# CycloneBoy/pdf_table

Measured on AMD Instinct MI355X. Metric: pages/s, higher is better.
Workload: dtype bf16

## Files before the change

include/pdftable_hip.h:

```cpp
#ifndef PDFTABLE_HIP_H
#define PDFTABLE_HIP_H

#include <stddef.h>
#include <stdint.h>

#ifdef __cplusplus
extern "C" {
#endif

#define PT_OK 0
#define PT_ERR_INVALID 1
#define PT_ERR_HIP 2
#define PT_ERR_STATE 3
#define PT_ERR_FORMAT 4

typedef struct pt_engine pt_engine;
typedef void* pt_stream;

int pt_engine_create(int device_id, pt_engine** out);
void pt_engine_destroy(pt_engine* e);
const char* pt_last_error(void);
int pt_abi_version(void);
int pt_engine_check(pt_engine* e);
int pt_engine_set_lstm_cluster(pt_engine* e, int on);
// ... 151 lines not shown
                  const float* d_cr, const float* d_reg, int n, int h, int w, int wiz_rev, float vis_thresh,
                  int32_t* d_counts, float* d_dets, float* d_logi, pt_stream stream);

int pt_tsr_forward_decode(pt_engine* e, const uint16_t* d_input_bf16, int n, int in_h, int in_w, int wiz_rev,
                          float vis_thresh, int32_t* d_counts, float* d_dets, float* d_logi, pt_stream stream);

int pt_centernet_forward_net(pt_engine* e, const uint16_t* d_input_bf16, int n, int H, int W, float* d_hm, float* d_v2c, float* d_c2v,
                             float* d_reg, pt_stream stream);

#define PT_CENTERNET_MAX_CELLS 1000
int pt_centernet_decode(pt_engine* e, const float* d_hm, const float* d_v2c, const float* d_c2v, const float* d_reg, int n, int h, int w,
                        const double* d_affine, int32_t* d_counts, float* d_cells, pt_stream stream);

int pt_tsr_process(pt_engine* e, const float* d_logi, const float* d_dets, const int32_t* h_counts, int n_tables,
                   int use_2dpe, float* d_logic, float* d_stacked, pt_stream stream);

int pt_op_conv2d(pt_engine* e, const uint16_t* d_in, int B, int H, int W, int Cin, const uint16_t* d_w_tiled,
                 const float* d_bias, int N, int ks, int stride, uint16_t* d_out, int out_cstride, int out_coff,
                 int rep, int shuffle_cout, const uint16_t* d_res, int res_mode, int relu, int split, int out_lo_off,
                 pt_stream stream);
int pt_op_conv1x1_ex(pt_engine* e, const uint16_t* d_in, int B, int H, int W, int Cin, const uint16_t* d_w_tiled, const float* d_bias,
                     int N, uint16_t* d_out, float* d_out_f32, int out_cstride, int n_valid, const float* d_res_f32, int relu,
                     const int32_t* d_ylimit, pt_stream stream);

int pt_op_dcn(pt_engine* e, const uint16_t* d_in, const float* d_om, int B, int H, int W, int C, const uint16_t* d_w_tiled,
              const float* d_bias, int N, uint16_t* d_out, int relu, int split, pt_stream stream);

int pt_op_stem7x7(pt_engine* e, const uint16_t* d_in, int B, int H, int W, const uint16_t* d_w, const float* d_bias,
                  uint16_t* d_out, int split, pt_stream stream);
int pt_op_maxpool3x3s2(pt_engine* e, const uint16_t* d_in, int B, int H, int W, int C, uint16_t* d_out, int split,
                       pt_stream stream);
int pt_op_db_head_final(pt_engine* e, const uint16_t* d_in, int B, int H, int W, const void* d_w, const float* d_bias,
                        float* d_prob, float* d_logits, int split, pt_stream stream);

int pt_op_dwconv(pt_engine* e, const uint16_t* d_in, int B, int H, int W, int C, const float* d_w_taps, const float* d_bias, int k,
                 int stride, int act, uint16_t* d_out, int split, pt_stream stream);
int pt_op_add(pt_engine* e, const uint16_t* d_a, const uint16_t* d_b, uint16_t* d_out, long long npix, int C, int split, pt_stream stream);
int pt_op_maxpool(pt_engine* e, const uint16_t* d_in, int B, int H, int W, int C, int k, int stride, int pad, uint16_t* d_out,
                  int split, pt_stream stream);
int pt_op_avgpool(pt_engine* e, const uint16_t* d_in, int B, int H, int W, int C, int k, uint16_t* d_out, int split, pt_stream stream);
int pt_op_chan_mean(pt_engine* e, const uint16_t* d_in, int B, int HW, int C, float* d_scratch, uint16_t* d_mean, int split, pt_stream stream);
int pt_op_chan_mean_scratch_floats(int B, int C);
int pt_op_scale_channels(pt_engine* e, const uint16_t* d_in, const uint16_t* d_gate, int B, int HW, int C, uint16_t* d_out,
                         int split, pt_stream stream);
int pt_op_act(pt_engine* e, const uint16_t* d_in, long long n_elems, int kind, float alpha, float beta, uint16_t* d_out, int C, int split,
              pt_stream stream);
// ... 73 lines not shown
```

pdf_table_amd/csrc/api_common.cpp:

```cpp
#include <stdarg.h>
#include <stdio.h>

#include "../../include/pdftable_hip.h"

static thread_local char g_err[1024] = "";

void pt_set_error(const char* fmt, ...) {
  va_list ap;
  va_start(ap, fmt);
  vsnprintf(g_err, sizeof(g_err), fmt, ap);
  va_end(ap);
}

extern "C" {

const char* pt_last_error(void) { return g_err; }

int pt_abi_version(void) { return 17; }

}
```

pdf_table_amd/csrc/c_api.hip:

```cpp
#include <stdarg.h>
#include <stdio.h>
#include <stdlib.h>

#include <cmath>

#include "common.h"

namespace PT_FMT_NS {
namespace api {

static int ensure(void** buf, size_t* cap, size_t need);

int pt_engine_check(pt_engine* e) {
  PT_REQUIRE(e, "pt_engine_check: null engine");
  if (e->lstm_err && *e->lstm_err) {
    *e->lstm_err = 0;
    e->lstm_cluster = 0;
    pt_set_error("lstm_cluster_kernel: a workgroup waited > 2^22 polls for its peers -- the launch was not co-resident "
                 "(GPU shared with another process or stream?).  The recognition results since the last check are invalid; "
                 "this engine now uses the streaming LSTM kernel (pt_engine_set_lstm_cluster(e, 0)): run the batch again");
    return PT_ERR_HIP;
  }
  return PT_OK;
}
// ... 910 lines not shown
                 const float* d_bias, int N, int ks, int stride, uint16_t* d_out, int out_cstride, int out_coff,
                 int rep, int shuffle_cout, const uint16_t* d_res, int res_mode, int relu, int split, int out_lo_off,
                 pt_stream stream) {
  PT_REQUIRE(e != nullptr, "pt_op_conv2d: null engine");
  ConvDesc d;
  d.in = d_in; d.B = B; d.H = H; d.W = W; d.Cin = Cin; d.w = d_w_tiled; d.bias = d_bias; d.N = N; d.ks = ks;
  d.stride = stride; d.out = d_out; d.out_cstride = out_cstride; d.out_coff = out_coff; d.rep = rep;
  d.shuffle_cout = shuffle_cout; d.res = d_res; d.res_mode = res_mode; d.relu = relu;
  d.split = split; d.out_lo_off = out_lo_off;
  return pt_launch_conv(e, d, reinterpret_cast<hipStream_t>(stream));
}

int pt_op_conv1x1_ex(pt_engine* e, const uint16_t* d_in, int B, int H, int W, int Cin, const uint16_t* d_w_tiled, const float* d_bias,
                     int N, uint16_t* d_out, float* d_out_f32, int out_cstride, int n_valid, const float* d_res_f32, int relu,
                     const int32_t* d_ylimit, pt_stream stream) {
  PT_REQUIRE(e != nullptr, "pt_op_conv1x1_ex: null engine");
  ConvDesc d;
  d.in = d_in; d.B = B; d.H = H; d.W = W; d.Cin = Cin; d.w = d_w_tiled; d.bias = d_bias; d.N = N; d.ks = 1; d.stride = 1;
  d.out = d_out_f32 ? nullptr : d_out; d.out_f32 = d_out_f32; d.out_cstride = out_cstride; d.n_valid = n_valid; d.res_f32 = d_res_f32;
  d.relu = relu; d.ylimit = d_ylimit;
  return pt_launch_conv(e, d, reinterpret_cast<hipStream_t>(stream));
}

int pt_op_stem7x7(pt_engine* e, const uint16_t* d_in, int B, int H, int W, const uint16_t* d_w, const float* d_bias,
                  uint16_t* d_out, int split, pt_stream stream) {
  PT_REQUIRE(e != nullptr, "pt_op_stem7x7: null engine");
  return pt_launch_stem7x7(e, d_in, B, H, W, d_w, d_bias, d_out, split, reinterpret_cast<hipStream_t>(stream));
}

int pt_op_maxpool3x3s2(pt_engine* e, const uint16_t* d_in, int B, int H, int W, int C, uint16_t* d_out, int split,
                       pt_stream stream) {
  PT_REQUIRE(e && d_in && d_out, "pt_op_maxpool3x3s2: bad arguments");
  return pt_launch_maxpool3x3s2(d_in, B, H, W, C, d_out, split, reinterpret_cast<hipStream_t>(stream));
}

int pt_op_db_head_final(pt_engine* e, const uint16_t* d_in, int B, int H, int W, const void* d_w, const float* d_bias,
                        float* d_prob, float* d_logits, int split, pt_stream stream) {
  PT_REQUIRE(e && d_in && d_w && d_bias && (d_prob || d_logits), "pt_op_db_head_final: bad arguments");
  return pt_launch_db_head_final(d_in, B, H, W, d_w, d_bias, d_prob, d_logits, split, reinterpret_cast<hipStream_t>(stream));
}

int pt_op_dcn(pt_engine* e, const uint16_t* d_in, const float* d_om, int B, int H, int W, int C, const uint16_t* d_w_tiled,
              const float* d_bias, int N, uint16_t* d_out, int relu, int split, pt_stream stream) {
  PT_REQUIRE(e && d_in && d_om && d_w_tiled && d_bias && d_out, "pt_op_dcn: null argument");
  PT_REQUIRE(B > 0 && H > 0 && W > 0, "pt_op_dcn: empty map (B=%d H=%d W=%d)", B, H, W);
  return pt_launch_dcn_fused(e, d_in, d_om, d_w_tiled, d_bias, d_out, B, H, W, C, N, split, relu, reinterpret_cast<hipStream_t>(stream));
// ... 86 lines not shown
```

pdf_table_amd/csrc/common.h:

```cpp
#pragma once
#include <hip/hip_runtime.h>
#include <stdint.h>
#include <string.h>

#include <map>
#include <string>
#include <vector>

#include "../../include/pdftable_hip.h"
#include "act16.h"

typedef uint16_t bf16_t;

void pt_set_error(const char* fmt, ...);

#define PT_HIP_CHECK(expr)                                                                  \
  do {                                                                                      \
    hipError_t _e = (expr);                                                                 \
    if (_e != hipSuccess) {                                                                 \
      pt_set_error("%s failed: %s (%s:%d)", #expr, hipGetErrorString(_e), __FILE__, __LINE__); \
      return PT_ERR_HIP;                                                                    \
    }                                                                                       \
  } while (0)

// ... 200 lines not shown
  const float* slope = nullptr;
  int pool = 0;
  const int* ylimit = nullptr;
  const int* xlimit = nullptr;
  const int* xlimit_cols = nullptr;
  const int* xlimit_rows = nullptr;
  const int* block_list = nullptr;
  int split = 0;
  int out_lo_off = 0;
  const void* head_w = nullptr;
  const float* head_b = nullptr;
  float* head_prob = nullptr;
  float* head_logits = nullptr;
  float* argmax_part = nullptr;
  int n_valid = 0;
  float* out_f32 = nullptr;
  const float* res_f32 = nullptr;
  unsigned tap_mask[8] = {0, 0, 0, 0, 0, 0, 0, 0};
  int xp_store = 0;
  int alg_n = 0;
  double alg_scale = 1.0;
};
int pt_launch_conv(pt_engine* e, const ConvDesc& d, hipStream_t s);
int pt_launch_crnn_conv01(pt_engine* e, const bf16_t* gray, int n, const float* w64x9, const float* b0, const bf16_t* w1, const float* b1, bf16_t* p1,
                          const int* xlimit, const int* xlimit_cols, hipStream_t s);
int pt_launch_dwpw(pt_engine* e, const bf16_t* in, int B, int H, int W, int C, const float* dw_w, const float* dw_b, int k, int stride, int dw_act,
                   const ConvDesc& pw, hipStream_t s);

int pt_launch_stem7x7(pt_engine* e, const bf16_t* in, int B, int H, int W, const bf16_t* w, const float* bias,
                      bf16_t* out, int split, hipStream_t s, int stride = 2, int n_valid = 0);

int pt_launch_det_preprocess(const uint8_t* pages, int n, int h, int w, int nh, int nw, int flavour, int split,
                             bf16_t* out, hipStream_t s);
int pt_launch_dcn_fused(pt_engine* e, const bf16_t* x, const float* om, const bf16_t* w, const float* bias, bf16_t* out,
                        int B, int H, int W, int C, int N, int split, int relu, hipStream_t s, const bf16_t* omw = nullptr, const float* omb = nullptr);
bool pt_dcn_fuses_om(const pt_engine* e, int C, int split);
int pt_launch_maxpool3x3s2(const bf16_t* in, int B, int H, int W, int C, bf16_t* out, int split, hipStream_t s);
int pt_launch_stem7x7_pool(pt_engine* e, const bf16_t* in, int B, int H, int W, const bf16_t* w, const float* bias, bf16_t* out,
                           hipStream_t s);
int pt_launch_db_head_final(const bf16_t* in, int B, int H, int W, const void* w4x64, const float* bias, float* prob,
                            float* logits, int split, hipStream_t s);
int pt_launch_db_head_mfma(const bf16_t* in, int B, int H, int W, const bf16_t* w3, const float* b3, const bf16_t* w6,
                           const float* b6, float* prob, float* logits, hipStream_t s, uint32_t* bitmap = nullptr, float thresh = 0.f);
int pt_launch_bitmap(const float* prob, int n, int H, int W, float thresh, int dilate, uint32_t* bitmap,
                     hipStream_t s);
int pt_launch_box_scores(const float* prob, int n, int H, int W, const float* boxes, int nb, float* scores,
// ... 149 lines not shown
```

pdf_table_amd/csrc/conv_igemm.hip:

```cpp
#include <stdio.h>
#include <stdlib.h>

#include <type_traits>

#include "common.h"

namespace PT_FMT_NS {

typedef __attribute__((ext_vector_type(8))) __bf16 bf16x8;
typedef __attribute__((ext_vector_type(8))) _Float16 f16x8;
typedef __attribute__((ext_vector_type(16))) float f32x16;
typedef __attribute__((ext_vector_type(4))) float f32x4;
typedef __attribute__((ext_vector_type(4))) uint32_t u32x4;
typedef __attribute__((ext_vector_type(2))) uint32_t u32x2;

struct ConvK {
  const bf16_t* in;
  const bf16_t* w;
  const float* bias;
  bf16_t* out;
  const bf16_t* res;
  int B, H, W, Cin, Ho, Wo, N;
  int out_cstride, out_coff, rep, shuffle_cout, res_mode, relu;
  int tiles_x, tiles_y, n_tiles;
// ... 1289 lines not shown
            stage[((rbase + m) * 32 + tx) * 64 + n * 32 + lx] = acc[m][n][r];
          }
    }
    __syncthreads();
    if constexpr (C::NBLK > 1) {
      static_assert(NT == 2 || C::NBLK == 1, "blocked tiles: one pass = all rows of one 64-channel half");
#pragma unroll 1
      for (int j = 0; j < C::NBLK; ++j) {
        int bj = blk_b[0], xj = blk_x[0];
#pragma unroll
        for (int t = 1; t < C::NBLK; ++t)
          if (j == t) { bj = blk_b[t]; xj = blk_x[t]; }
        if (xj < p.Wo) epilogue_store<C::BR, 32, C::NTHR, 2>(p, stage + j * C::BR * 32 * 64, tid, bj, 0, xj, (nb * 2 + pass) * 64);
      }
    } else if (NT == 1) {
      epilogue_store<C::PASS_ROWS, 32, C::NTHR, 0>(p, stage, tid, b, oy0 + C::PASS_ROWS * pass, ox0, nb * 64);
    } else {
      epilogue_store<C::PASS_ROWS, 32, C::NTHR, 0>(p, stage, tid, b, oy0, ox0, (nb * 2 + pass) * 64);
    }
  }
#endif
}

template <int NT, int NWV, int S>
__global__ __launch_bounds__(64 * NWV, 2) void conv3x3_pipe_persist_kernel(ConvK p) {
#if defined(__HIP_DEVICE_COMPILE__)
  a16_kernel_enter();
  using C = PipeCfg<NT, NWV, 0, S>;
  static_assert(C::NBLK == 1, "ordinary tiles");
  extern __shared__ __attribute__((aligned(16))) char smem[];
  const int tid = threadIdx.x;
  const int lane = tid & 63;
  const int wave = __builtin_amdgcn_readfirstlane(tid >> 6);
  const int lx = lane & 31, qh = lane >> 5;
  const int wm = NT == 1 ? wave : (wave >> 1);
  const int wn = NT == 1 ? 0 : (wave & 1);
  const int G = gridDim.x;
  const int Lw = xcd_remap(blockIdx.x, G);
  const int t0 = (int)((long long)Lw * p.total_tiles / G), t1 = (int)((long long)(Lw + 1) * p.total_tiles / G);
  if (t0 >= t1) return;
  const int in_cs = p.Cin;
  const int nch32 = p.Cin >> 5, nslices = nch32 * 2;

  constexpr int OOB = 0x7FFFF000;
  int meta[C::SLOTS];
  bool is_in[C::SLOTS];
  int dst[C::SLOTS];
#pragma unroll
  for (int j = 0; j < C::SLOTS; ++j) {
    int k = wave + NWV * j;
    if (k >= C::T_INSTR) k = C::T_INSTR - 1;
    is_in[j] = k < C::IN_INSTR;
    dst[j] = k * 1024;
    if (is_in[j]) {
      const int U = k * 64 + lane;
      const int pix = U >> 1;
      const int pr = pix / C::TWIN, sx = pix - pr * C::TWIN;
      const int q = (U & 1) ^ ((sx >> 3) & 1);
      const int ix = S == 1 ? sx : (sx < C::XEVEN ? 2 * sx : 2 * (sx - C::XEVEN) + 1);
      meta[j] = U < C::IN_UNITS ? (pr | (ix << 8) | (q << 16)) : -1;
    } else {
      const int U = (k - C::IN_INSTR) * 64 + lane;
// ... 102 lines not shown
      __syncthreads();
      if constexpr (!LAST) load_frags(smem + (P ^ 1) * C::BUF_BYTES, 0, ((P + 1) * NTAP) & 1);
      mma_tap((P * NTAP + NTAP - 1) & 1);
      tap_groups<LAST ? 0 : 2 + C::MT, 2 * C::MT, 0>();
    };
    for (int c = 0; c + 2 < nslices; c += 2) {
      skew_slice(c, std::integral_constant<int, 0>{}, std::false_type{}, in_off(c + 1), w_off(c + 1));
      skew_slice(c + 1, std::integral_constant<int, 1>{}, std::false_type{}, in_off(c + 2), w_off(c + 2));
    }
    skew_slice(nslices - 2, std::integral_constant<int, 0>{}, std::false_type{}, in_off(nslices - 1), w_off(nslices - 1));
    const Tile done = cur;
    {
      const bool has_next = ti + 1 < t1;
      cur = decode(has_next ? ti + 1 : ti);
      offsets(cur, vo);
      if (!has_next) {
#pragma unroll
        for (int j = 0; j < C::SLOTS; ++j) vo[j] = OOB;
      }
      r_in = rsrc_in(cur);
      r_w = rsrc_w(cur);
    }
    skew_slice(nslices - 1, std::integral_constant<int, 1>{}, std::true_type{}, 0, 0);
    {
      const int n0 = (NT == 1 ? done.nb : done.nb * 2 + wn) * 64;
      const DirectBias bs = direct_bias<2>(p, n0, qh);
#pragma unroll
      for (int m = 0; m < C::MT; ++m) {
        epilogue_direct_row<2>(p, acc[m], bs, done.b, done.oy0 + C::MT * wm + m, done.ox0, lx, n0, qh, nullptr);
#pragma unroll
        for (int n = 0; n < 2; ++n)
#pragma unroll
          for (int r = 0; r < 16; ++r) acc[m][n][r] = 0.f;
      }
    }
    load_frags(smem, 0, 0);
  }
#endif
}

struct GemmPipeCfg {
  static constexpr int NWV = 8, NTHR = 512, MT = 4, NG = 16;
  static constexpr int KS = 64, NW = 128;
  static constexpr int A_BYTES = NG * 32 * KS * 2, W_BYTES = NW * KS * 2, BUF_BYTES = A_BYTES + W_BYTES;
  static constexpr int A_INSTR = A_BYTES / 1024, W_INSTR = W_BYTES / 1024, SLOTS = (A_INSTR + W_INSTR) / NWV;
  static constexpr int SMEM = 2 * BUF_BYTES;
  static_assert(A_INSTR % NWV == 0 && W_INSTR % NWV == 0, "a slot is an A or a W request for every wave alike");
};

template <bool LIST>
__global__ __launch_bounds__(512, 2) void gemm_pipe_kernel(ConvK p) {
#if defined(__HIP_DEVICE_COMPILE__)
  a16_kernel_enter();
  using C = GemmPipeCfg;
  extern __shared__ __attribute__((aligned(16))) char smem[];
  const int tid = threadIdx.x;
  const int lane = tid & 63;
  const int wave = __builtin_amdgcn_readfirstlane(tid >> 6);
  const int lx = lane & 31, qh = lane >> 5;
  const int wm = wave >> 1, wn = wave & 1;

// ... 1435 lines not shown
  k.n_tiles = k.N / C::NW;
  k.tiles_x = (k.Wo + C::TW - 1) / C::TW;
  k.tiles_y = (k.Ho + C::TH - 1) / C::TH;
  const long long total = (long long)k.B * k.tiles_x * k.tiles_y * k.n_tiles;
  PT_REQUIRE(total > 0 && total < (1ll << 31), "conv grid out of range (%lld tiles)", total);
  k.total_tiles = (int)total;
  const int per_cu = 2 * C::BUF_BYTES <= 80 * 1024 ? 2 : 1;
  long long grid = (long long)e->num_cu * per_cu;
  if (const char* gv = getenv("PT_CONV_PERSIST_GRID")) {
    const int gg = atoi(gv);
    if (gg > 0) grid = gg;
  }
  if (grid > total) grid = total;
  char label[48];
  snprintf(label, sizeof(label), "conv3x3 %sv5%s %d->%d @%dx%d", S == 2 ? "s2 " : "", NWV == 4 ? "h" : "", k.Cin, k.N, k.Ho, k.Wo);
  {
    PtProfScope prof(e, s, PT_PROF_CONV3X3, flop, label);
    hipLaunchKernelGGL((conv3x3_pipe_persist_kernel<NT, NWV, S>), dim3((unsigned)grid), dim3(C::NTHR), 2 * C::BUF_BYTES, s, k);
  }
  PT_HIP_CHECK(hipGetLastError());
  return PT_OK;
}

static int launch_gemm_pipe(pt_engine* e, ConvK& k, hipStream_t s, double flop) {
  using C = GemmPipeCfg;
  static bool attr_done = false;
  if (!attr_done) {
    PT_HIP_CHECK(hipFuncSetAttribute(reinterpret_cast<const void*>(&gemm_pipe_kernel<false>), hipFuncAttributeMaxDynamicSharedMemorySize, C::SMEM));
    PT_HIP_CHECK(hipFuncSetAttribute(reinterpret_cast<const void*>(&gemm_pipe_kernel<true>), hipFuncAttributeMaxDynamicSharedMemorySize, C::SMEM));
    attr_done = true;
  }
  const long long M = (long long)k.B * k.H * k.W, groups = M / 32;
  {
    const char* xv = getenv("PT_GEMM_XP");
    k.xp_store = !(xv && xv[0] == '0') && !k.out_f32;
  }
  k.n_tiles = k.N / C::NW;
  k.tiles_x = (int)((groups + C::NG - 1) / C::NG);
  k.tiles_y = 1;
  const long long nblk = (long long)k.tiles_x * k.n_tiles;
  PT_REQUIRE(nblk > 0 && nblk < (1ll << 31), "gemm grid out of range (%lld blocks)", nblk);
  char label[48];
  if (k.argmax_part) snprintf(label, sizeof(label), "classifier gemm+argmax");
  else snprintf(label, sizeof(label), "gemm %d->%d @%dx%d", k.Cin, k.N, k.Ho, k.Wo);
  int lim_slot = -1;
  {
// ... 386 lines not shown
```

pdf_table_amd/csrc/dla_net.h:

```cpp
#pragma once

#include <stdlib.h>

#include <string>
#include <vector>

#include "net_ctx.h"

namespace PT_FMT_NS {

int pt_launch_conv3x3_c16(pt_engine* e, const bf16_t* in, const bf16_t* w, const float* bias, bf16_t* out, int B, int H, int W,
                          int N, int stride, int split, hipStream_t s);
int pt_launch_dla_thin_chain(pt_engine* e, const bf16_t* in, int B, int H, int W, const bf16_t* w_stem, const float* b_stem, const bf16_t* w0,
                             const float* b0, const bf16_t* w1, const float* b1, bf16_t* out, hipStream_t s);

namespace {

struct DlaCtx : NetCtx {
  bf16_t* cols = nullptr;
  float* om = nullptr;
  const int* ylimit = nullptr;
  double alg_scale = 1.0;

  void conv(const T& in, const std::string& q, int N, int ks, int stride, const T& out, int relu, const T* res = nullptr,
// ... 23 lines not shown
    c.w = W(w); c.bias = F(b);
    c.N = N; c.ks = 1; c.stride = 1; c.relu = relu; c.split = x3; c.alg_scale = alg_scale;
    to_map(c, out);
    launch(c);
  }
  T maxpool2(const T& x) {
    T o = alloc(x.H / 2, x.W / 2, x.C);
    if (go()) {
      e->prof.next_bytes = (double)n * x.H * x.W * x.C * 2.0 * mul * 1.25;
      PtProfScope ps(e, s, PT_PROF_OTHER, 0, "maxpool2x2");
      const int r = pt_launch_maxpool_kxk(x.p, n, x.H, x.W, x.C, 2, 2, 0, x3, o.p, s);
      if (r != PT_OK) rc = r;
    }
    return o;
  }
  T block(const std::string& q, const T& x, const T& residual, int stride, int cout) {
    T t = alloc(x.H / stride, x.W / stride, cout);
    conv(x, q + ".conv1", cout, 3, stride, t, 1);
    T o = alloc(t.H, t.W, cout);
    conv(t, q + ".conv2", cout, 3, 1, o, 1, &residual);
    return o;
  }
  T tree(const std::string& q, int levels, const T& x, int cin, int cout, int stride, bool level_root,
         std::vector<T> children) {
    T bottom = stride > 1 ? maxpool2(x) : x;
    if (level_root) children.push_back(bottom);
    if (levels == 1) {
      T residual = bottom;
      if (cin != cout) {
        residual = alloc(bottom.H, bottom.W, cout);
        conv(bottom, q + ".project", cout, 1, 1, residual, 0);
      }
      T x1 = block(q + ".tree1", x, residual, stride, cout);
      T x2 = block(q + ".tree2", x1, x1, 1, cout);
      std::vector<T> ins = {x2, x1};
      ins.insert(ins.end(), children.begin(), children.end());
      T o = alloc(x1.H, x1.W, cout);
      conv_cat(ins, q + ".root", cout, o, 1);
      return o;
    }
    T x1 = tree(q + ".tree1", levels - 1, x, cin, cout, stride, false, {});
    children.push_back(x1);
    return tree(q + ".tree2", levels - 1, x1, cout, cout, 1, false, children);
  }
};

static std::vector<T> dla34_base(DlaCtx& c, const bf16_t* x, int H, int W) {
  pt_engine* e = c.e;
  hipStream_t s = c.s;
  const int n = c.n;
  const int ch[6] = {16, 32, 64, 128, 256, 512};
  const int lv[6] = {1, 1, 1, 2, 2, 1};
  const char* chain_env = getenv("PT_DLA_CHAIN");
  const bool chain = !c.x3 && H % 2 == 0 && W % 2 == 0 && !(chain_env && atoi(chain_env) == 0);
  std::vector<T> layers(6);
  if (chain) {
    layers[1] = c.alloc(H / 2, W / 2, 32);
    const PtTensor *ws = c.get("base_layer.w"), *bs = c.get("base_layer.b"), *w0 = c.get("level0.wt"), *b0 = c.get("level0.bt"),
                   *w1 = c.get("level1.wt"), *b1 = c.get("level1.bt");
    if (c.go()) {
      const int r = pt_launch_dla_thin_chain(e, x, n, H, W, c.W(ws), c.F(bs), c.W(w0), c.F(b0), c.W(w1), c.F(b1), layers[1].p, s);
      if (r != PT_OK) c.rc = r;
    }
  } else {
// ... 29 lines not shown
```

pdf_table_amd/csrc/lore_kernels.hip:

```cpp
#include <stdio.h>
#include <stdlib.h>

#include "common.h"

namespace PT_FMT_NS {

typedef __attribute__((ext_vector_type(4))) uint32_t u32x4;
typedef __attribute__((ext_vector_type(2))) uint32_t u32x2;

namespace {

__device__ __forceinline__ float bf2f(uint32_t b) { return a16_to_f32(b); }
__device__ __forceinline__ uint32_t f2bf(float f) { return f32_to_a16(f); }

__device__ __forceinline__ void load8(const bf16_t* p, int lo_off, int split, float* v) {
  const u32x4 h = *reinterpret_cast<const u32x4*>(p);
  const uint32_t hw[4] = {h.x, h.y, h.z, h.w};
#pragma unroll
  for (int k = 0; k < 8; ++k) v[k] = bf2f((k & 1) ? (hw[k >> 1] >> 16) : (hw[k >> 1] & 0xFFFFu));
  if (split) {
    const u32x4 l = *reinterpret_cast<const u32x4*>(p + lo_off);
    const uint32_t lw[4] = {l.x, l.y, l.z, l.w};
#pragma unroll
    for (int k = 0; k < 8; ++k) v[k] += bf2f((k & 1) ? (lw[k >> 1] >> 16) : (lw[k >> 1] & 0xFFFFu));
// ... 254 lines not shown
  const int wt[4] = {(32 - ay) * (32 - ax) * 32, (32 - ay) * ax * 32, ay * (32 - ax) * 32, ay * ax * 32};
  int acc[3] = {0, 0, 0};
  const uint8_t* pg = pages + (size_t)tb.page * ph * pw * 3;
#pragma unroll
  for (int k = 0; k < 4; ++k) {
    const long long yy = sy + (k >> 1), xx = sx + (k & 1);
    if (yy < 0 || yy >= tb.crop_h || xx < 0 || xx >= tb.crop_w) continue;
    const long long py = tb.y0 + yy, px = tb.x0 + xx;
    if (py < 0 || py >= ph || px < 0 || px >= pw) continue;
    const uint8_t* s = pg + ((size_t)py * pw + px) * 3;
    acc[0] += s[0] * wt[k]; acc[1] += s[1] * wt[k]; acc[2] += s[2] * wt[k];
  }
  float v[3];
#pragma unroll
  for (int c = 0; c < 3; ++c) {
    const int sc = bgr ? 2 - c : c;
    int u = (acc[sc] + (1 << 14)) >> 15;
    u = u < 0 ? 0 : (u > 255 ? 255 : u);
    v[c] = lut[c * 256 + u];
  }
  bf16_t* o = out + ((size_t)t * H * W + i) * (split ? 8 : 4);
  uint32_t hb[3];
#pragma unroll
  for (int c = 0; c < 3; ++c) { hb[c] = f2bf(v[c]); o[c] = (bf16_t)hb[c]; }
  o[3] = 0;
  if (split) {
#pragma unroll
    for (int c = 0; c < 3; ++c) o[4 + c] = (bf16_t)f2bf(v[c] - bf2f(hb[c]));
    o[7] = 0;
  }
}

typedef __attribute__((ext_vector_type(8))) __bf16 dbf16x8;
typedef __attribute__((ext_vector_type(16))) float df32x16;
typedef __attribute__((ext_vector_type(2))) float df2;
__device__ __forceinline__ uint32_t pack_df2(df2 v) { return pack_a16x2(v.x, v.y); }
__device__ __forceinline__ df2 unpack_df2(uint32_t pk) { return df2{a16lo_f32(pk), a16hi_f32(pk)}; }

template <int SPLIT, int NB>
__global__ __launch_bounds__(256, (SPLIT || NB > 64) ? 2 : 4) void dcn_fused_kernel(const bf16_t* __restrict__ x, const float* __restrict__ om,
                                                            const bf16_t* __restrict__ w, const float* __restrict__ bias,
                                                            bf16_t* __restrict__ out, long long npix, int H, int W, int C,
                                                            int N, int relu) {
#pragma clang fp contract(fast)
  a16_kernel_enter();
  constexpr int ROW = 80;
  constexpr int NP = SPLIT ? 2 : 1;
  constexpr int NT = NB / 32;
  __shared__ __attribute__((aligned(16))) char s_a[NP][128 * ROW];
  __shared__ __attribute__((aligned(16))) char s_w[NP][NB * ROW];
  const int tid = threadIdx.x, lane = tid & 63, wave = tid >> 6;
  const int lx = lane & 31, q = lane >> 5;
// ... 1580 lines not shown
```

pdf_table_amd/csrc/lore_model.hip:

```cpp
#include "dla_net.h"

namespace PT_FMT_NS {

int pt_launch_dcn_im2col(const bf16_t* x, const float* om, bf16_t* cols, int B, int H, int W, int C, int split,
                         hipStream_t s);
int pt_launch_dwconvt_up_add(const bf16_t* in, const float* w, const bf16_t* add, bf16_t* out, int B, int h, int wd,
                             int C, int f, int split, hipStream_t s);

namespace {

struct Ctx : DlaCtx {
  T dcn(const std::string& q, const T& x, int cout) {
    T o = alloc(x.H, x.W, cout);
    static const bool fused = !(getenv("PT_DCN_FUSED") && atoi(getenv("PT_DCN_FUSED")) == 0);
    const bool om_inside = fused && pt_dcn_fuses_om(e, x.C, x3);
    if (!om_inside) conv(x, q + ".om", 64, 3, 1, T(), 0, nullptr, 32, om, 32, 0, 27);
    if (fused) {
      const PtTensor* w = get(q + (x3 ? ".dcn.w3" : ".dcn.w"));
      const PtTensor* b = get(q + ".dcn.b");
      const PtTensor* ow = om_inside ? get(q + (x3 ? ".om.w3" : ".om.w")) : nullptr;
      const PtTensor* ob = om_inside ? get(q + ".om.b") : nullptr;
      if (go()) {
        const int r = pt_launch_dcn_fused(e, x.p, om, W(w), F(b), o.p, n, x.H, x.W, x.C, cout, x3, 1, s, ow ? W(ow) : nullptr, ob ? F(ob) : nullptr);
        if (r != PT_OK) rc = r;
// ... 52 lines not shown
  const char* hname[6] = {"hm", "st", "wh", "ax", "cr", "reg"};
  const int hcs[6] = {8, 8, 8, 256, 256, 8};
  const int hreal[6] = {2, 8, 8, 256, 256, 2};

  return pt_plan_then_launch(c, "Lore net", [&]() -> int {
    const size_t px4 = (size_t)n * (H / 4) * (W / 4);
    c.cols = c.take<bf16_t>(px4 * 576 * c.mul * sizeof(bf16_t));
    c.om = c.take<float>(px4 * 32 * sizeof(float));

    std::vector<T> layers = dla34_base(c, x, H, W);

    std::vector<T> out = {layers[5]};
    const int f2[4] = {1, 2, 2, 2};
    c.ida("dla_up.ida_0", layers, 4, 6, 256, f2);
    out.insert(out.begin(), layers[5]);
    c.ida("dla_up.ida_1", layers, 3, 6, 128, f2);
    out.insert(out.begin(), layers[5]);
    c.ida("dla_up.ida_2", layers, 2, 6, 64, f2);
    out.insert(out.begin(), layers[5]);
    std::vector<T> y = {out[0], out[1], out[2]};
    const int f24[3] = {1, 2, 4};
    c.ida("ida_up", y, 0, 3, 64, f24);
    const T feat = y[2];
    T hid = c.alloc(feat.H, feat.W, 256);
    if (sp) heads[0] = c.take<float>((size_t)n * feat.H * feat.W * 8 * sizeof(float));
    for (int h = 0; h < 6; ++h) {
      if (sp && h != 0) continue;
      c.conv(feat, std::string(hname[h]) + ".0", 256, 3, 1, hid, 1);
      c.conv(hid, std::string(hname[h]) + ".2", hcs[h] < 64 ? 64 : hcs[h], 1, 1, T(), 0, nullptr, hcs[h], heads[h], hcs[h], 0, hreal[h]);
    }
    if (sp) {
      int rows_ax = 0, rows_cr = 0, rows_cell = 0, rows_corner = 0;
      pt_lore_mosaic_rows(n, &rows_ax, &rows_cr, &rows_cell, &rows_corner);
      const int MW = 32;
      auto mosaic = [&](int rows, int C) {
        T t;
        t.H = rows; t.W = MW; t.C = C;
        t.p = c.take<bf16_t>(((size_t)rows * MW * C * c.mul + 64) * sizeof(bf16_t));
        return t;
      };
      T mcell = mosaic(rows_cell, 9 * 64), mcorner = mosaic(rows_corner, 9 * 64), max_ = mosaic(rows_ax, 9 * 64), mcr_ = mosaic(rows_cr, 9 * 64);
      T mhid = mosaic(rows_cr, 256);
      float* o_wh = c.take<float>((size_t)rows_cell * MW * 8 * sizeof(float));
      float* o_regc = c.take<float>((size_t)rows_cell * MW * 8 * sizeof(float));
      float* o_st = c.take<float>((size_t)rows_corner * MW * 8 * sizeof(float));
      float* o_regk = c.take<float>((size_t)rows_corner * MW * 8 * sizeof(float));
      float* oax = c.take<float>((size_t)rows_ax * MW * 256 * sizeof(float));
      float* ocr = c.take<float>((size_t)rows_cr * MW * 256 * sizeof(float));
      if (c.go()) {
        const int keep = c.n;
// ... 140 lines not shown
```

pdf_table_amd/engine.py:

```python
from __future__ import annotations

import contextlib
import ctypes as C
import functools
import threading
from typing import Optional, Sequence, Tuple

import numpy as np
import torch

from . import lib as L

__all__ = ["HipEngine", "REC_LINE_DTYPE", "CLS_IMAGE_DTYPE", "REC_PP_ITEM_DTYPE"]

TSR_TABLE_DTYPE = np.dtype([("minv", "<f8", (6,)), ("page", "<i4"), ("x0", "<i4"), ("y0", "<i4"),
                            ("crop_w", "<i4"), ("crop_h", "<i4"), ("reserved", "<i4")])
CLS_IMAGE_DTYPE = np.dtype([("offset", "<i8"), ("h", "<i4"), ("w", "<i4")])
REC_LINE_DTYPE = np.dtype([("minv", np.float64, (9,)), ("page", np.int32), ("crop_w", np.int32), ("crop_h", np.int32),
                           ("reserved", np.int32)])


REC_PP_ITEM_DTYPE = np.dtype([("line", "<i4"), ("resized_w", "<i4"), ("img_w", "<i4"), ("reserved", "<i4"),
                              ("out_off", "<i8")])

# ... 606 lines not shown
        if out is None:
            if shuffle_cout:
                out = torch.empty((B, 2 * Ho, 2 * Wo, shuffle_cout * m), dtype=self.act_dtype, device=self._tdev)
            else:
                out = torch.empty((B, Ho * rep, Wo * rep, N * m), dtype=self.act_dtype, device=self._tdev)
        L.check(self.lib.pt_op_conv2d(self._h, _ptr(x), B, H, W, Cin, _ptr(w_tiled), _ptr(bias), N, ks, stride,
                                      _ptr(out), out.shape[-1], out_coff, rep, shuffle_cout, _ptr(res), res_mode,
                                      int(relu), int(split), out.shape[-1] // 2, self._stream()), "pt_op_conv2d")
        return out

    def op_conv1x1_ex(self, x: torch.Tensor, w_tiled: torch.Tensor, bias: torch.Tensor, relu: int = 0, out_f32: bool = False,
                      n_valid: int = 0, res_f32: Optional[torch.Tensor] = None, ylimit: Optional[torch.Tensor] = None) -> torch.Tensor:
        self._chk(x, self.act_dtype, "x")
        self._chk(bias, torch.float32, "bias")
        B, H, W, Cin = x.shape
        N = bias.numel()
        cs = n_valid or N
        out = torch.zeros((B, H, W, cs), dtype=torch.float32 if out_f32 else self.act_dtype, device=self._tdev)
        L.check(self.lib.pt_op_conv1x1_ex(self._h, _ptr(x), B, H, W, Cin, _ptr(w_tiled), _ptr(bias), N, None if out_f32 else _ptr(out),
                                          _ptr(out) if out_f32 else None, cs, n_valid, _ptr(res_f32), int(relu), _ptr(ylimit),
                                          self._stream()), "pt_op_conv1x1_ex")
        return out

    def op_dcn(self, x: torch.Tensor, om: torch.Tensor, w_tiled: torch.Tensor, bias: torch.Tensor, relu: bool = True, split: int = 0) -> torch.Tensor:
        self._chk(x, self.act_dtype, "x")
        self._chk(om, torch.float32, "om")
        self._chk(bias, torch.float32, "bias")
        B, H, W, Cc = x.shape
        m = 2 if split else 1
        Cc //= m
        if tuple(om.shape) != (B, H, W, 32):
            raise ValueError(f"op_dcn: om must be [B,H,W,32], got {tuple(om.shape)}")
        N = bias.numel()
        out = torch.empty((B, H, W, N * m), dtype=self.act_dtype, device=self._tdev)
        L.check(self.lib.pt_op_dcn(self._h, _ptr(x), _ptr(om), B, H, W, Cc, _ptr(w_tiled), _ptr(bias), N, _ptr(out), int(relu), int(split),
                                   self._stream()), "pt_op_dcn")
        return out

    def op_dwconv(self, x: torch.Tensor, w_taps: torch.Tensor, bias: torch.Tensor, k: int, stride: int = 1, act: int = 0, split: bool = False) -> torch.Tensor:
        self._chk(x, self.act_dtype, "x")
        self._chk(w_taps, torch.float32, "w_taps")
        self._chk(bias, torch.float32, "bias")
        B, H, W, Cc = x.shape
        pad = k // 2
        out = torch.empty((B, (H + 2 * pad - k) // stride + 1, (W + 2 * pad - k) // stride + 1, Cc), dtype=self.act_dtype, device=self._tdev)
        L.check(self.lib.pt_op_dwconv(self._h, _ptr(x), B, H, W, Cc // 2 if split else Cc, _ptr(w_taps), _ptr(bias), k, stride, act, _ptr(out), int(split),
# ... 270 lines not shown
```

pdf_table_amd/lib.py:

```python
from __future__ import annotations

import ctypes as C
import os

_HERE = os.path.dirname(os.path.abspath(__file__))
LIB_PATH = os.environ.get("PT_LIB_PATH") or os.path.join(_HERE, "libpdftable_hip.so")

PT_MODEL_DB_RESNET18 = 1
PT_MODEL_CRNN = 2
PT_MODEL_LORE_DLA34 = 3
PT_MODEL_LORE_PROCESSOR = 4
PT_MODEL_PICODET = 5
PT_MODEL_LORE_RESNET18 = 6
PT_MODEL_DB_NAS = 7
PT_MODEL_PPLCNET = 8
PT_MODEL_CONVNEXT_VIT = 16
PT_MODEL_MTL_BACKBONE = 17
PT_MODEL_MTL_DECODER = 18
PT_MODEL_CENTERNET_DLA34 = 19
PT_CVIT_W, PT_CVIT_CHUNK_W, PT_CVIT_CHUNK_STEP, PT_CVIT_T, PT_CVIT_NCLS = 804, 300, 252, 201, 7644
PT_CLS_SLOTS = 4
PT_CLS_MAX_CLASSES = 16
PT_LAYOUT_HEAD_CS, PT_LAYOUT_CAND_FLOATS = 40, 48
PT_DET_PRE_DB_PP = 0
PT_DET_PRE_DB_TORCH = 1
PT_DET_PRE_NONE = 2
PT_PRECISION_BF16 = 0
PT_PRECISION_BF16X3 = 1
PT_PRECISION_F16X2 = 2
PT_PRECISION_F16 = 3
PT_DET_POST_DB_PP = 0
PT_DET_POST_DB_TORCH = 1
PT_TSR_MAX_CELLS = 3000
PT_CENTERNET_MAX_CELLS = 1000
PT_ROTATE_90_CLOCKWISE, PT_ROTATE_180, PT_ROTATE_90_COUNTERCLOCKWISE = 0, 1, 2
PT_REC_H, PT_REC_W, PT_REC_T, PT_REC_NCLS = 32, 640, 160, 7644
PT_PROF_CLASSES = ("conv3x3", "conv1x1", "stem", "other")
EXPECTED_ABI = 17

_lib = None


class PtError(RuntimeError):
    pass


def _proto(lib):
    vp, i, f, sz = C.c_void_p, C.c_int, C.c_float, C.c_size_t
    ip = C.POINTER(C.c_int)
    P = {
        "pt_engine_create": (i, [i, C.POINTER(vp)]),
        "pt_engine_destroy": (None, [vp]),
        "pt_last_error": (C.c_char_p, []),
        "pt_abi_version": (i, []),
        "pt_engine_check": (i, [vp]),
        "pt_engine_set_precision": (i, [vp, i]),
        "pt_engine_set_lstm_cluster": (i, [vp, i]),
        "pt_engine_set_mtl_kv_fp8": (i, [vp, i]),
        "pt_engine_set_dcn_mfma": (i, [vp, i]),
        "pt_weights_load": (i, [vp, i, vp, sz]),
        "pt_weights_load_device": (i, [vp, i, vp, sz, vp]),
# ... 29 lines not shown
        "pt_layout_candidates": (i, [vp, vp, vp, vp, vp, i, i, i, i, f, i, vp, vp, vp]),
        "pt_layout_forward": (i, [vp, vp, i, i, i, i, i, i, f, i, vp, vp, vp]),
        "pt_tsr_preprocess": (i, [vp, vp, i, i, i, vp, i, i, i, i, vp, vp]),
        "pt_tsr_forward_net": (i, [vp, vp, i, i, i, vp, vp, vp, vp, vp, vp, vp]),
        "pt_tsr_forward_net_wireless": (i, [vp, vp, i, i, i, vp, vp, vp, vp, vp, vp, vp]),
        "pt_tsr_decode": (i, [vp, vp, vp, vp, vp, vp, vp, i, i, i, i, f, vp, vp, vp, vp]),
        "pt_tsr_forward_decode": (i, [vp, vp, i, i, i, i, f, vp, vp, vp, vp]),
        "pt_tsr_process": (i, [vp, vp, vp, vp, i, i, vp, vp, vp]),
        "pt_centernet_forward_net": (i, [vp, vp, i, i, i, vp, vp, vp, vp, vp]),
        "pt_centernet_decode": (i, [vp, vp, vp, vp, vp, i, i, i, vp, vp, vp, vp]),
        "pt_hard_nms": (i, [vp, vp, vp, i, C.c_double, i, vp, vp]),
        "pt_page_line_mask": (i, [vp, i, i, i, vp, vp]),
        "pt_page_line_angles": (i, [vp, i, i, i, i, i, vp, i, vp]),
        "pt_page_warp_cubic": (i, [vp, i, i, i, vp, vp, i, vp, vp]),
        "pt_page_quarter_turn": (i, [vp, i, i, i, i, vp, vp]),
        "pt_page_pre_tables": (i, [vp, vp]),
        "pt_cls_preprocess": (i, [vp, vp, vp, i, i, i, i, i, vp, vp]),
        "pt_cls_forward_net": (i, [vp, i, vp, i, i, i, i, vp, ip, vp]),
        "pt_cls_forward": (i, [vp, i, vp, vp, i, i, i, i, i, i, vp, ip, vp]),
        "pt_cls_forward_lines": (i, [vp, i, vp, i, i, i, vp, vp, i, i, i, i, i, i, vp, ip, vp]),
        "pt_cls_forward_lines_direct": (i, [vp, i, vp, i, i, i, vp, i, i, i, i, i, i, vp, ip, vp]),
        "pt_op_conv2d": (i, [vp, vp, i, i, i, i, vp, vp, i, i, i, vp, i, i, i, i, vp, i, i, i, i, vp]),
        "pt_op_conv1x1_ex": (i, [vp, vp, i, i, i, i, vp, vp, i, vp, vp, i, i, vp, i, vp, vp]),
        "pt_op_dcn": (i, [vp, vp, vp, i, i, i, i, vp, vp, i, vp, i, i, vp]),
        "pt_op_stem7x7": (i, [vp, vp, i, i, i, vp, vp, vp, i, vp]),
        "pt_op_maxpool3x3s2": (i, [vp, vp, i, i, i, i, vp, i, vp]),
        "pt_op_db_head_final": (i, [vp, vp, i, i, i, vp, vp, vp, vp, i, vp]),
        "pt_op_dwconv": (i, [vp, vp, i, i, i, i, vp, vp, i, i, i, vp, i, vp]),
        "pt_op_add": (i, [vp, vp, vp, vp, C.c_longlong, i, i, vp]),
        "pt_op_maxpool": (i, [vp, vp, i, i, i, i, i, i, i, vp, i, vp]),
        "pt_op_avgpool": (i, [vp, vp, i, i, i, i, i, vp, i, vp]),
        "pt_op_chan_mean": (i, [vp, vp, i, i, i, vp, vp, i, vp]),
        "pt_op_chan_mean_scratch_floats": (i, [i, i]),
        "pt_op_scale_channels": (i, [vp, vp, vp, i, i, i, vp, i, vp]),
        "pt_op_act": (i, [vp, vp, C.c_longlong, i, C.c_float, C.c_float, vp, i, i, vp]),
        "pt_op_copy_channels": (i, [vp, vp, C.c_longlong, i, i, vp, i, i, i, vp]),
        "pt_op_upsample_nearest": (i, [vp, vp, i, i, i, i, i, vp, vp]),
        "pt_op_mul": (i, [vp, vp, vp, vp, C.c_longlong, i, i, vp]),
        "pt_copy_bytes": (i, [vp, vp, vp, C.c_longlong, vp]),
        "pt_op_layernorm": (i, [vp, vp, C.c_longlong, i, i, vp, vp, C.c_float, vp, i, vp]),
        "pt_op_softmax": (i, [vp, vp, C.c_longlong, i, i, vp, vp, i, vp]),
        "pt_op_attention": (i, [vp, vp, i, i, i, i, i, C.c_float, vp, i, i, vp]),
        "pt_op_lstm": (i, [vp, vp, i, vp, i, i, i, i, i, vp, i, i, vp]),
        "pt_op_lstm_packed_elems": (i, [i, i, i]),
        "pt_profile_enable": (i, [vp, i]),
        "pt_profile_read": (i, [vp, vp, vp, vp]),
# ... 34 lines not shown
```

Before: 809.0.

## Fuse LORE head 3x3 conv with 1x1 projection; pool once in DLA trees

Adds a fused kernel that computes the 256-channel 3x3 hidden layer of each 8-channel LORE head and immediately applies the 1x1 output projection on the hidden tile held in registers. The two 128-channel halves are chained through LDS to accumulate the result. This avoids writing the 256-channel hidden activation to memory, reading it back, and launching a second kernel. It also reuses the max-pooled tensor across DLA tree recursion instead of pooling twice, and vectorizes the packed preprocess store. In exchange it adds an extra __syncthreads per tile pair and assigns tiles in pairs, which can unbalance the persistent grid.

Result: no change. 805.4 (-0.5%).

```diff
diff --git a/include/pdftable_hip.h b/include/pdftable_hip.h
--- a/include/pdftable_hip.h
+++ b/include/pdftable_hip.h
@@ -197,6 +197,8 @@
 int pt_op_conv1x1_ex(pt_engine* e, const uint16_t* d_in, int B, int H, int W, int Cin, const uint16_t* d_w_tiled, const float* d_bias,
                      int N, uint16_t* d_out, float* d_out_f32, int out_cstride, int n_valid, const float* d_res_f32, int relu,
                      const int32_t* d_ylimit, pt_stream stream);
+int pt_op_conv3x3_head(pt_engine* e, const uint16_t* d_in, int B, int H, int W, int Cin, const uint16_t* d_w1_tiled, const float* d_b1,
+                       const uint16_t* d_w2_tiled, const float* d_b2, int nc_real, float* d_out, int out_cstride, pt_stream stream);
 
 int pt_op_dcn(pt_engine* e, const uint16_t* d_in, const float* d_om, int B, int H, int W, int C, const uint16_t* d_w_tiled,
               const float* d_bias, int N, uint16_t* d_out, int relu, int split, pt_stream stream);
diff --git a/pdf_table_amd/csrc/api_common.cpp b/pdf_table_amd/csrc/api_common.cpp
--- a/pdf_table_amd/csrc/api_common.cpp
+++ b/pdf_table_amd/csrc/api_common.cpp
@@ -16,6 +16,6 @@
 
 const char* pt_last_error(void) { return g_err; }
 
-int pt_abi_version(void) { return 17; }
+int pt_abi_version(void) { return 18; }
 
 }
diff --git a/pdf_table_amd/csrc/c_api.hip b/pdf_table_amd/csrc/c_api.hip
--- a/pdf_table_amd/csrc/c_api.hip
+++ b/pdf_table_amd/csrc/c_api.hip
@@ -956,6 +956,12 @@
   return pt_launch_conv(e, d, reinterpret_cast<hipStream_t>(stream));
 }
 
+int pt_op_conv3x3_head(pt_engine* e, const uint16_t* d_in, int B, int H, int W, int Cin, const uint16_t* d_w1_tiled, const float* d_b1,
+                       const uint16_t* d_w2_tiled, const float* d_b2, int nc_real, float* d_out, int out_cstride, pt_stream stream) {
+  PT_REQUIRE(e != nullptr, "pt_op_conv3x3_head: null engine");
+  return pt_launch_conv3x3_head(e, d_in, B, H, W, Cin, d_w1_tiled, d_b1, d_w2_tiled, d_b2, nc_real, d_out, out_cstride, reinterpret_cast<hipStream_t>(stream));
+}
+
 int pt_op_stem7x7(pt_engine* e, const uint16_t* d_in, int B, int H, int W, const uint16_t* d_w, const float* d_bias,
                   uint16_t* d_out, int split, pt_stream stream) {
   PT_REQUIRE(e != nullptr, "pt_op_stem7x7: null engine");
diff --git a/pdf_table_amd/csrc/common.h b/pdf_table_amd/csrc/common.h
--- a/pdf_table_amd/csrc/common.h
+++ b/pdf_table_amd/csrc/common.h
@@ -246,6 +246,8 @@
   double alg_scale = 1.0;
 };
 int pt_launch_conv(pt_engine* e, const ConvDesc& d, hipStream_t s);
+int pt_launch_conv3x3_head(pt_engine* e, const bf16_t* in, int B, int H, int W, int Cin, const bf16_t* w1, const float* b1, const bf16_t* w2,
+                           const float* b2, int nc_real, float* out, int out_cs, hipStream_t s);
 int pt_launch_crnn_conv01(pt_engine* e, const bf16_t* gray, int n, const float* w64x9, const float* b0, const bf16_t* w1, const float* b1, bf16_t* p1,
                           const int* xlimit, const int* xlimit_cols, hipStream_t s);
 int pt_launch_dwpw(pt_engine* e, const bf16_t* in, int B, int H, int W, int C, const float* dw_w, const float* dw_b, int k, int stride, int dw_act,
diff --git a/pdf_table_amd/csrc/conv_igemm.hip b/pdf_table_amd/csrc/conv_igemm.hip
--- a/pdf_table_amd/csrc/conv_igemm.hip
+++ b/pdf_table_amd/csrc/conv_igemm.hip
@@ -1335,10 +1335,9 @@
 #endif
 }
 
-template <int NT, int NWV, int S>
-__global__ __launch_bounds__(64 * NWV, 2) void conv3x3_pipe_persist_kernel(ConvK p) {
+template <int NT, int NWV, int S, bool HEAD>
+__device__ __forceinline__ void conv3x3_pipe_persist_body(const ConvK& p) {
 #if defined(__HIP_DEVICE_COMPILE__)
-  a16_kernel_enter();
   using C = PipeCfg<NT, NWV, 0, S>;
   static_assert(C::NBLK == 1, "ordinary tiles");
   extern __shared__ __attribute__((aligned(16))) char smem[];
@@ -1350,7 +1349,9 @@
   const int wn = NT == 1 ? 0 : (wave & 1);
   const int G = gridDim.x;
   const int Lw = xcd_remap(blockIdx.x, G);
-  const int t0 = (int)((long long)Lw * p.total_tiles / G), t1 = (int)((long long)(Lw + 1) * p.total_tiles / G);
+  static_assert(!HEAD || (NT == 2 && S == 1), "fused head: 128-channel halves of a 256-channel hidden layer");
+  const int run_unit = HEAD ? 2 : 1, nrun = p.total_tiles / run_unit;
+  const int t0 = (int)((long long)Lw * nrun / G) * run_unit, t1 = (int)((long long)(Lw + 1) * nrun / G) * run_unit;
   if (t0 >= t1) return;
   const int in_cs = p.Cin;
   const int nch32 = p.Cin >> 5, nslices = nch32 * 2;
@@ -1499,7 +1500,65 @@
       r_w = rsrc_w(cur);
     }
     skew_slice(nslices - 1, std::integral_constant<int, 1>{}, std::true_type{}, 0, 0);
-    {
+    if constexpr (HEAD) {
+      const int n0 = (done.nb * 2 + wn) * 64;
+      bf16x8 wf[4];
+#pragma unroll
+      for (int j = 0; j < 4; ++j) {
+        const int ks = (n0 >> 4) + j;
+        wf[j] = *reinterpret_cast<const bf16x8*>(reinterpret_cast<const bf16_t*>(p.head_w) + (ks >> 1) * (64 * 32) + lx * 32 + (ks & 1) * 16 + qh * 8);
+      }
+      const DirectBias bs = direct_bias<2>(p, n0, qh);
+      u32x4 hf[C::MT][4];
+#pragma unroll
+      for (int m = 0; m < C::MT; ++m)
+#pragma unroll
+        for (int nb = 0; nb < 2; ++nb) {
+          uint32_t d[8];
+#pragma unroll
+          for (int k = 0; k < 8; ++k) {
+            const int g = k >> 1, c = (k & 1) * 2;
+            d[k] = pack_bf16x2(fmaxf(acc[m][nb][4 * g + c] + bs.v[nb][g][c], 0.f), fmaxf(acc[m][nb][4 * g + c + 1] + bs.v[nb][g][c + 1], 0.f));
+          }
+          const u32x2 s0 = __builtin_amdgcn_permlane32_swap(d[0], d[2], false, false);
+          const u32x2 s1 = __builtin_amdgcn_permlane32_swap(d[1], d[3], false, false);
+          const u32x2 s2 = __builtin_amdgcn_permlane32_swap(d[4], d[6], false, false);
+          const u32x2 s3 = __builtin_amdgcn_permlane32_swap(d[5], d[7], false, false);
+          hf[m][2 * nb] = u32x4{s0.x, s1.x, s0.y, s1.y};
+          hf[m][2 * nb + 1] = u32x4{s2.x, s3.x, s2.y, s3.y};
+#pragma unroll
+          for (int r = 0; r < 16; ++r) acc[m][nb][r] = 0.f;
+        }
+      float* chain = reinterpret_cast<float*>(smem + 2 * C::BUF_BYTES) + wm * (C::MT * 4 * 64) + lane;
+      auto link = [&]() {
+        const int step = done.nb * 2 + wn;
+        const f32x4 b2 = *reinterpret_cast<const f32x4*>(p.head_b + 4 * qh);
+#pragma unroll
+        for (int m = 0; m < C::MT; ++m) {
+          f32x16 a2;
+#pragma unroll
+          for (int r = 0; r < 16; ++r) a2[r] = 0.f;
+          if (step > 0) {
+#pragma unroll
+            for (int r = 0; r < 4; ++r) a2[r] = chain[(m * 4 + r) * 64];
+          }
+#pragma unroll
+          for (int j = 0; j < 4; ++j) a2 = mfma_32x32x16_a16(wf[j], __builtin_bit_cast(bf16x8, hf[m][j]), a2);
+          if (step < 3) {
+#pragma unroll
+            for (int r = 0; r < 4; ++r) chain[(m * 4 + r) * 64] = a2[r];
+          } else {
+            const int oy = done.oy0 + C::MT * wm + m, ox = done.ox0 + lx;
+            if (oy < p.Ho && ox < p.Wo)
+              *reinterpret_cast<f32x4*>(p.out_f32 + (((size_t)done.b * p.Ho + oy) * p.Wo + ox) * p.out_cstride + 4 * qh) =
+                  f32x4{a2[0] + b2.x, a2[1] + b2.y, a2[2] + b2.z, a2[3] + b2.w};
+          }
+        }
+      };
+      if (wn == 0) link();
+      __syncthreads();
+      if (wn == 1) link();
+    } else {
       const int n0 = (NT == 1 ? done.nb : done.nb * 2 + wn) * 64;
       const DirectBias bs = direct_bias<2>(p, n0, qh);
 #pragma unroll
@@ -1514,6 +1573,15 @@
     load_frags(smem, 0, 0);
   }
 #endif
+}
+template <int NT, int NWV, int S>
+__global__ __launch_bounds__(64 * NWV, 2) void conv3x3_pipe_persist_kernel(ConvK p) {
+  a16_kernel_enter();
+  conv3x3_pipe_persist_body<NT, NWV, S, false>(p);
+}
+__global__ __launch_bounds__(512, 2) void conv3x3_head_kernel(ConvK p) {
+  a16_kernel_enter();
+  conv3x3_pipe_persist_body<2, 8, 1, true>(p);
 }
 
 struct GemmPipeCfg {
@@ -2995,6 +3063,48 @@
   return PT_OK;
 }
 
+int pt_launch_conv3x3_head(pt_engine* e, const bf16_t* in, int B, int H, int W, int Cin, const bf16_t* w1, const float* b1, const bf16_t* w2,
+                           const float* b2, int nc_real, float* out, int out_cs, hipStream_t s) {
+  using C = PipeCfg<2, 8, 0, 1>;
+  constexpr int SMEM = 2 * C::BUF_BYTES + 4 * C::MT * 4 * 64 * 4;
+  static_assert(SMEM <= 163840, "LDS budget");
+  PT_REQUIRE(in && w1 && b1 && w2 && b2 && out, "conv3x3 head: null pointer");
+  PT_REQUIRE(B > 0 && H > 0 && W > 0 && Cin > 0 && Cin % 32 == 0, "conv3x3 head: bad input shape (B=%d H=%d W=%d Cin=%d)", B, H, W, Cin);
+  PT_REQUIRE(nc_real > 0 && nc_real <= 8 && out_cs >= 8 && out_cs % 4 == 0, "conv3x3 head: nc_real=%d out_cs=%d unsupported", nc_real, out_cs);
+  PT_REQUIRE(!pt_split(e), "conv3x3 head: single-pass precisions only");
+  static bool attr_done = false;
+  if (!attr_done) {
+    PT_HIP_CHECK(hipFuncSetAttribute(reinterpret_cast<const void*>(&conv3x3_head_kernel), hipFuncAttributeMaxDynamicSharedMemorySize, SMEM));
+    attr_done = true;
+  }
+  ConvK k;
+  memset(&k, 0, sizeof(k));
+  k.in = in; k.w = w1; k.bias = b1; k.head_w = w2; k.head_b = b2; k.out_f32 = out; k.out_cstride = out_cs;
+  k.B = B; k.H = H; k.W = W; k.Cin = Cin; k.Ho = H; k.Wo = W; k.N = 256; k.relu = 1; k.rep = 1;
+  k.n_tiles = 2;
+  k.tiles_x = (W + C::TW - 1) / C::TW;
+  k.tiles_y = (H + C::TH - 1) / C::TH;
+  const long long pairs = (long long)B * k.tiles_x * k.tiles_y;
+  PT_REQUIRE(pairs < (1ll << 30), "conv grid out of range (%lld tiles)", 2 * pairs);
+  k.total_tiles = (int)(2 * pairs);
+  long long grid = e->num_cu;
+  if (const char* gv = getenv("PT_CONV_PERSIST_GRID")) {
+    const int gg = atoi(gv);
+    if (gg > 0) grid = gg;
+  }
+  if (grid > pairs) grid = pairs;
+  const double px = (double)B * H * W;
+  e->prof.next_bytes = px * Cin * 2.0 + px * nc_real * 4.0 + (256.0 * Cin * 9 + 256.0 * nc_real) * 2.0;
+  char label[48];
+  snprintf(label, sizeof(label), "conv3x3 v5+head %d->256->%d @%dx%d", Cin, nc_real, H, W);
+  {
+    PtProfScope prof(e, s, PT_PROF_CONV3X3, 2.0 * px * 9 * Cin * 256 + 2.0 * px * 256 * nc_real, label);
+    hipLaunchKernelGGL(conv3x3_head_kernel, dim3((unsigned)grid), dim3(C::NTHR), SMEM, s, k);
+  }
+  PT_HIP_CHECK(hipGetLastError());
+  return PT_OK;
+}
+
 static int launch_gemm_pipe(pt_engine* e, ConvK& k, hipStream_t s, double flop) {
   using C = GemmPipeCfg;
   static bool attr_done = false;
diff --git a/pdf_table_amd/csrc/dla_net.h b/pdf_table_amd/csrc/dla_net.h
--- a/pdf_table_amd/csrc/dla_net.h
+++ b/pdf_table_amd/csrc/dla_net.h
@@ -69,8 +69,8 @@
     return o;
   }
   T tree(const std::string& q, int levels, const T& x, int cin, int cout, int stride, bool level_root,
-         std::vector<T> children) {
-    T bottom = stride > 1 ? maxpool2(x) : x;
+         std::vector<T> children, const T* pooled = nullptr) {
+    T bottom = stride > 1 ? (pooled ? *pooled : maxpool2(x)) : x;
     if (level_root) children.push_back(bottom);
     if (levels == 1) {
       T residual = bottom;
@@ -86,7 +86,9 @@
       conv_cat(ins, q + ".root", cout, o, 1);
       return o;
     }
-    T x1 = tree(q + ".tree1", levels - 1, x, cin, cout, stride, false, {});
+    const char* once_env = getenv("PT_DLA_POOL_ONCE");
+    const bool once = stride > 1 && !(once_env && atoi(once_env) == 0);
+    T x1 = tree(q + ".tree1", levels - 1, x, cin, cout, stride, false, {}, once ? &bottom : nullptr);
     children.push_back(x1);
     return tree(q + ".tree2", levels - 1, x1, cout, cout, 1, false, children);
   }
diff --git a/pdf_table_amd/csrc/lore_kernels.hip b/pdf_table_amd/csrc/lore_kernels.hip
--- a/pdf_table_amd/csrc/lore_kernels.hip
+++ b/pdf_table_amd/csrc/lore_kernels.hip
@@ -300,12 +300,15 @@
   bf16_t* o = out + ((size_t)t * H * W + i) * (split ? 8 : 4);
   uint32_t hb[3];
 #pragma unroll
-  for (int c = 0; c < 3; ++c) { hb[c] = f2bf(v[c]); o[c] = (bf16_t)hb[c]; }
-  o[3] = 0;
+  for (int c = 0; c < 3; ++c) hb[c] = f2bf(v[c]) & 0xFFFFu;
+  const uint32_t h01 = hb[0] | (hb[1] << 16), h2 = hb[2];
   if (split) {
-#pragma unroll
-    for (int c = 0; c < 3; ++c) o[4 + c] = (bf16_t)f2bf(v[c] - bf2f(hb[c]));
-    o[7] = 0;
+    uint32_t lb[3];
+#pragma unroll
+    for (int c = 0; c < 3; ++c) lb[c] = f2bf(v[c] - bf2f(hb[c])) & 0xFFFFu;
+    *reinterpret_cast<uint4*>(o) = make_uint4(h01, h2, lb[0] | (lb[1] << 16), lb[2]);
+  } else {
+    *reinterpret_cast<uint2*>(o) = make_uint2(h01, h2);
   }
 }
 
diff --git a/pdf_table_amd/csrc/lore_model.hip b/pdf_table_amd/csrc/lore_model.hip
--- a/pdf_table_amd/csrc/lore_model.hip
+++ b/pdf_table_amd/csrc/lore_model.hip
@@ -98,10 +98,22 @@
     const int f24[3] = {1, 2, 4};
     c.ida("ida_up", y, 0, 3, 64, f24);
     const T feat = y[2];
-    T hid = c.alloc(feat.H, feat.W, 256);
+    const char* hf_env = getenv("PT_LORE_HEAD_FUSED");
+    const bool head_fused = !c.x3 && !(hf_env && atoi(hf_env) == 0);
+    T hid;
+    if (!head_fused || !sp) hid = c.alloc(feat.H, feat.W, 256);
     if (sp) heads[0] = c.take<float>((size_t)n * feat.H * feat.W * 8 * sizeof(float));
     for (int h = 0; h < 6; ++h) {
       if (sp && h != 0) continue;
+      if (head_fused && hcs[h] == 8) {
+        const std::string q = hname[h];
+        const PtTensor *w1 = c.get(q + ".0.w"), *b1 = c.get(q + ".0.b"), *w2 = c.get(q + ".2.w"), *b2 = c.get(q + ".2.b");
+        if (c.go()) {
+          const int r = pt_launch_conv3x3_head(e, feat.p, n, feat.H, feat.W, feat.C, c.W(w1), c.F(b1), c.W(w2), c.F(b2), hreal[h], heads[h], hcs[h], s);
+          if (r != PT_OK) c.rc = r;
+        }
+        continue;
+      }
       c.conv(feat, std::string(hname[h]) + ".0", 256, 3, 1, hid, 1);
       c.conv(hid, std::string(hname[h]) + ".2", hcs[h] < 64 ? 64 : hcs[h], 1, 1, T(), 0, nullptr, hcs[h], heads[h], hcs[h], 0, hreal[h]);
     }
diff --git a/pdf_table_amd/engine.py b/pdf_table_amd/engine.py
--- a/pdf_table_amd/engine.py
+++ b/pdf_table_amd/engine.py
@@ -652,6 +652,17 @@
                                           self._stream()), "pt_op_conv1x1_ex")
         return out
 
+    def op_conv3x3_head(self, x: torch.Tensor, w1_tiled: torch.Tensor, b1: torch.Tensor, w2_tiled: torch.Tensor, b2: torch.Tensor,
+                        nc_real: int, out_cs: int = 8) -> torch.Tensor:
+        self._chk(x, self.act_dtype, "x")
+        self._chk(b1, torch.float32, "b1")
+        self._chk(b2, torch.float32, "b2")
+        B, H, W, Cin = x.shape
+        out = torch.zeros((B, H, W, out_cs), dtype=torch.float32, device=self._tdev)
+        L.check(self.lib.pt_op_conv3x3_head(self._h, _ptr(x), B, H, W, Cin, _ptr(w1_tiled), _ptr(b1), _ptr(w2_tiled), _ptr(b2), int(nc_real),
+                                            _ptr(out), out_cs, self._stream()), "pt_op_conv3x3_head")
+        return out
+
     def op_dcn(self, x: torch.Tensor, om: torch.Tensor, w_tiled: torch.Tensor, bias: torch.Tensor, relu: bool = True, split: int = 0) -> torch.Tensor:
         self._chk(x, self.act_dtype, "x")
         self._chk(om, torch.float32, "om")
diff --git a/pdf_table_amd/lib.py b/pdf_table_amd/lib.py
--- a/pdf_table_amd/lib.py
+++ b/pdf_table_amd/lib.py
@@ -36,7 +36,7 @@
 PT_ROTATE_90_CLOCKWISE, PT_ROTATE_180, PT_ROTATE_90_COUNTERCLOCKWISE = 0, 1, 2
 PT_REC_H, PT_REC_W, PT_REC_T, PT_REC_NCLS = 32, 640, 160, 7644
 PT_PROF_CLASSES = ("conv3x3", "conv1x1", "stem", "other")
-EXPECTED_ABI = 17
+EXPECTED_ABI = 18
 
 _lib = None
 
@@ -112,6 +112,7 @@
         "pt_cls_forward_lines_direct": (i, [vp, i, vp, i, i, i, vp, i, i, i, i, i, i, vp, ip, vp]),
         "pt_op_conv2d": (i, [vp, vp, i, i, i, i, vp, vp, i, i, i, vp, i, i, i, i, vp, i, i, i, i, vp]),
         "pt_op_conv1x1_ex": (i, [vp, vp, i, i, i, i, vp, vp, i, vp, vp, i, i, vp, i, vp, vp]),
+        "pt_op_conv3x3_head": (i, [vp, vp, i, i, i, i, vp, vp, vp, vp, i, vp, i, vp]),
         "pt_op_dcn": (i, [vp, vp, vp, i, i, i, i, vp, vp, i, vp, i, i, vp]),
         "pt_op_stem7x7": (i, [vp, vp, i, i, i, vp, vp, vp, i, vp]),
         "pt_op_maxpool3x3s2": (i, [vp, vp, i, i, i, i, vp, i, vp]),
```
